# neuronika/neuronika

Hardware: AMD Instinct MI355X
Metric: training-step samples/sec (fwd+bwd+allreduce) (higher is better)
Workload: dtype f32

## Files before the change

neuronika_amd/csrc/nk_gemm.hip:

```cpp
#include "nk_mma.h"
#include <utility>

using namespace nkmma;

static bool aligned16(const void* p) { return (reinterpret_cast<uintptr_t>(p) & 15) == 0; }
constexpr int GEMM_CHAIN_K = 2048;
constexpr int PF2_MIN_KTILES = 48;

struct GemmArgs {
    const float* A;
    const float* B;
    float* C;
    int M, N, K;
    long long lda, ldb, ldc;
    float alpha, beta;
    const float* bias;
    int relu;
    const float* mask;
    long long ldm;
    int batch_inner;
    long long sAo, sAi, sBo, sBi, sCo, sCi;
    int splits;
    int k_per_split;
    float* slabs;
    int tiles_m, tiles_n;
    int chunk;
    int group_m;
    int pf2_min;
    int kskew;
};

template <bool ALIGNED, int TI, int TJ, bool EPX>
__device__ __forceinline__ void gemm_epilogue(const GemmArgs& p, f32x16 (&acc)[TI][TJ], int m0, int n0, int bo, int bi, int split,
                                              int batch, int wr, int wc, int lane) {
    if (p.splits > 1) {
        float* S = p.slabs + ((long long)split * gridDim.z + batch) * (long long)p.M * p.N;
        const int M = p.M, N = p.N;
        acc_foreach<TI, TJ>(acc, wr, wc, lane, [&](int r, int c, float v) {
            const int row = m0 + r, col = n0 + c;
            if (ALIGNED || (row < M && col < N)) S[(long long)row * N + col] = v;
        });
        return;
    }
    float* C = p.C + bo * p.sCo + bi * p.sCi;
    const float alpha = p.alpha, beta = p.beta;
    const int M = p.M, N = p.N;
    const long long ldc = p.ldc;
    if (EPX && p.mask != nullptr) {
        const float* Mk = p.mask;
        const long long ldm = p.ldm;
#pragma unroll
        for (int i = 0; i < TI; ++i)
#pragma unroll
            for (int j = 0; j < TJ; ++j) {
                float mv[16], old[16];
#pragma unroll
                for (int e = 0; e < 16; ++e) {
                    const int row = m0 + (wr * TI + i) * 32 + (e & 3) + 8 * (e >> 2) + 4 * (lane >> 5), col = n0 + (wc * TJ + j) * 32 + (lane & 31);
                    const bool ok = ALIGNED || (row < M && col < N);
                    mv[e] = ok ? Mk[row * ldm + col] : 0.f;
                    old[e] = (ok && beta != 0.f) ? C[row * ldc + col] : 0.f;
                }
#pragma unroll
                for (int e = 0; e < 16; ++e) {
                    const int row = m0 + (wr * TI + i) * 32 + (e & 3) + 8 * (e >> 2) + 4 * (lane >> 5), col = n0 + (wc * TJ + j) * 32 + (lane & 31);
                    float o = alpha * acc[i][j][e];
                    o = mv[e] > 0.f ? o : 0.f * o;
                    if (ALIGNED || (row < M && col < N)) C[row * ldc + col] = beta == 0.f ? o : fmaf(beta, old[e], o);
                }
            }
        return;
    }
    if (p.bias != nullptr || beta != 0.f || alpha != 1.f || (EPX && p.relu)) {
        float old[TI][TJ][16];
        if (beta != 0.f)
            acc_foreach_idx<TI, TJ>(acc, wr, wc, lane, [&](int i, int j, int e, int r, int c, float) {
                const int row = m0 + r, col = n0 + c;
                old[i][j][e] = (ALIGNED || (row < M && col < N)) ? C[row * ldc + col] : 0.f;
            });
        float bv[TJ];
#pragma unroll
        for (int j = 0; j < TJ; ++j) {
            const int col = n0 + (wc * TJ + j) * 32 + (lane & 31);
            bv[j] = (p.bias != nullptr && (ALIGNED || col < N)) ? p.bias[col] : 0.f;
        }
        const bool relu = EPX && p.relu != 0;
#pragma unroll
        for (int i = 0; i < TI; ++i)
#pragma unroll
            for (int j = 0; j < TJ; ++j)
#pragma unroll
                for (int e = 0; e < 16; ++e) {
                    float o = alpha * acc[i][j][e];
                    if (p.bias != nullptr) o += bv[j];
                    if constexpr (EPX) o = relu ? fmaxf(o, 0.f) : o;
                    acc[i][j][e] = beta == 0.f ? o : fmaf(beta, old[i][j][e], o);
                }
    }
    acc_foreach<TI, TJ>(acc, wr, wc, lane, [&](int r, int c, float v) {
        const int row = m0 + r, col = n0 + c;
        if (ALIGNED || (row < M && col < N)) C[row * ldc + col] = v;
    });
}

template <bool AKC, bool BKC, bool ALIGNED, int TI, int TJ, int KG>
__device__ __forceinline__ void gemm_loop_lookahead2(TileLoader<AKC, 64 * TI>& la, TileLoader<BKC, 64 * TJ>& lb, f32x16 (&acc)[TI][TJ],
                                                     float* smem, int nt, bool skew, int t, int wr, int wc, int lane) {
    constexpr int BM = 64 * TI, BN = 64 * TJ;
    constexpr int TA_FLOATS = tile_floats<AKC, BM>(), STAGE = TA_FLOATS + tile_floats<BKC, BN>();
    float* const buf0 = smem;
    float* const buf1 = smem + STAGE;
    Stage<BM / 32> pa, qa;
    Stage<BN / 32> pb, qb;
    if (nt > 0) {
        pa = la.template load<ALIGNED>(t);
        pb = lb.template load<ALIGNED>(t);
        stage_store<AKC, BM>(buf0, pa, t);
        stage_store<BKC, BN>(buf0 + TA_FLOATS, pb, t);
    }
    __syncthreads();
    if (nt > 1) {
        pa = la.template load<ALIGNED>(t);
        pb = lb.template load<ALIGNED>(t);
    }
    int it = 0;
    for (; it + 3 < nt; it += 2) {
        if (KG == 2 && skew) {
            mma_tile<AKC, BKC, TI, TJ, 0, BK / 16>(buf0, buf0 + TA_FLOATS, acc, wr, wc, lane);
            __builtin_amdgcn_sched_barrier(0);
        }
        qa = la.template load<ALIGNED>(t);
        qb = lb.template load<ALIGNED>(t);
        stage_store<AKC, BM>(buf1, pa, t);
        stage_store<BKC, BN>(buf1 + TA_FLOATS, pb, t);
        __builtin_amdgcn_sched_barrier(0);
        if (KG == 2 && skew) mma_tile<AKC, BKC, TI, TJ, BK / 16, BK / 8>(buf0, buf0 + TA_FLOATS, acc, wr, wc, lane);
        else mma_tile<AKC, BKC, TI, TJ>(buf0, buf0 + TA_FLOATS, acc, wr, wc, lane);
        __syncthreads();
        if (KG == 2 && skew) {
            mma_tile<AKC, BKC, TI, TJ, 0, BK / 16>(buf1, buf1 + TA_FLOATS, acc, wr, wc, lane);
            __builtin_amdgcn_sched_barrier(0);
        }
        pa = la.template load<ALIGNED>(t);
        pb = lb.template load<ALIGNED>(t);
        stage_store<AKC, BM>(buf0, qa, t);
        stage_store<BKC, BN>(buf0 + TA_FLOATS, qb, t);
        __builtin_amdgcn_sched_barrier(0);
        if (KG == 2 && skew) mma_tile<AKC, BKC, TI, TJ, BK / 16, BK / 8>(buf1, buf1 + TA_FLOATS, acc, wr, wc, lane);
        else mma_tile<AKC, BKC, TI, TJ>(buf1, buf1 + TA_FLOATS, acc, wr, wc, lane);
        __syncthreads();
    }
    const int left = nt - it;
    if (left == 3) {
        qa = la.template load<ALIGNED>(t);
        qb = lb.template load<ALIGNED>(t);
    }
    if (left >= 2) {
        stage_store<AKC, BM>(buf1, pa, t);
        stage_store<BKC, BN>(buf1 + TA_FLOATS, pb, t);
    }
    if (left >= 1) mma_tile<AKC, BKC, TI, TJ>(buf0, buf0 + TA_FLOATS, acc, wr, wc, lane);
    if (left >= 2) {
        __syncthreads();
        if (left == 3) {
            stage_store<AKC, BM>(buf0, qa, t);
            stage_store<BKC, BN>(buf0 + TA_FLOATS, qb, t);
        }
        mma_tile<AKC, BKC, TI, TJ>(buf1, buf1 + TA_FLOATS, acc, wr, wc, lane);
        if (left == 3) {
            __syncthreads();
            mma_tile<AKC, BKC, TI, TJ>(buf0, buf0 + TA_FLOATS, acc, wr, wc, lane);
        }
    }
}

template <bool TA, bool TB, int TI, int TJ, int KG>
constexpr int gemm_smem_floats() { return KG * 2 * (tile_floats<!TA, 64 * TI>() + tile_floats<TB, 64 * TJ>()); }

template <bool TA, bool TB, bool ALIGNED, int TI, int TJ, int KG = 1, bool EPX = false>
__global__ __launch_bounds__(NT * KG, (min_waves<TI, TJ, !TA && TB>())) void sgemm_kernel(GemmArgs p) {
    __shared__ __attribute__((aligned(16))) float smem_all[gemm_smem_floats<TA, TB, TI, TJ, KG>()];
#define NK_GEMM_BX blockIdx.x
#define NK_GEMM_NBX gridDim.x
#define NK_GEMM_SPLIT blockIdx.y
#include "nk_gemm_body.h"
#undef NK_GEMM_BX
#undef NK_GEMM_NBX
#undef NK_GEMM_SPLIT
}

template <bool TA, bool TB, bool ALIGNED, int TI, int TJ, int KG, bool EPX>
__device__ __forceinline__ void sgemm_body(const GemmArgs& p, float* smem_all, int bx, int nbx) {
#define NK_GEMM_BX bx
#define NK_GEMM_NBX nbx
#define NK_GEMM_SPLIT blockIdx.y
#include "nk_gemm_body.h"
#undef NK_GEMM_BX
#undef NK_GEMM_NBX
#undef NK_GEMM_SPLIT
}
template <bool TA, bool TB, bool ALIGNED, int TI, int TJ, int KG, bool EPX>
__device__ __forceinline__ void sgemm_body_split(const GemmArgs& p, float* smem_all, int bx, int nbx, int split_no) {
#define NK_GEMM_BX bx
#define NK_GEMM_NBX nbx
#define NK_GEMM_SPLIT split_no
#include "nk_gemm_body.h"
#undef NK_GEMM_BX
#undef NK_GEMM_NBX
#undef NK_GEMM_SPLIT
}

struct GemmPairArgs {
    GemmArgs p0, p1;
    int nblk0;
};
template <bool TA0, bool TB0, bool TA1, bool TB1, int TI, int TJ>
__global__ __launch_bounds__(NT, (min_waves<TI, TJ, (!TA0 && TB0) || (!TA1 && TB1)>())) void sgemm_pair_kernel(GemmPairArgs pp) {
    constexpr int F0 = gemm_smem_floats<TA0, TB0, TI, TJ, 1>(), F1 = gemm_smem_floats<TA1, TB1, TI, TJ, 1>();
    __shared__ __attribute__((aligned(16))) float smem_all[F0 > F1 ? F0 : F1];
    const int nblk0 = pp.nblk0;
    if ((int)blockIdx.x < nblk0)
        sgemm_body<TA0, TB0, true, TI, TJ, 1, false>(pp.p0, smem_all, blockIdx.x, nblk0);
    else
        sgemm_body<TA1, TB1, true, TI, TJ, 1, false>(pp.p1, smem_all, blockIdx.x - nblk0, gridDim.x - nblk0);
}

struct GemmTailArgs {
    GemmArgs p0, p1;
    int nfull, ntail;
};
template <bool TA, bool TB, bool EPX>
__global__ __launch_bounds__(NT, (min_waves<2, 2, !TA && TB>())) void sgemm_tail_kernel(GemmTailArgs pp) {
    __shared__ __attribute__((aligned(16))) float smem_all[gemm_smem_floats<TA, TB, 2, 2, 1>()];
    const int nfull = pp.nfull;
    if ((int)blockIdx.x < nfull) {
        sgemm_body_split<TA, TB, true, 2, 2, 1, EPX>(pp.p0, smem_all, blockIdx.x, nfull, 0);
    } else {
        const int r = (int)blockIdx.x - nfull, ntail = pp.ntail;
        sgemm_body_split<TA, TB, true, 2, 2, 1, false>(pp.p1, smem_all, r % ntail, ntail, r / ntail);
    }
}

__global__ void splitk_reduce_kernel(const float* __restrict__ slabs, float* __restrict__ C, int M, int N,
                                     long long ldc, int splits, int nbatch, int batch_inner,
                                     long long sCo, long long sCi, float alpha, float beta,
                                     const float* __restrict__ bias, int relu, const float* __restrict__ mask, long long ldm) {
    const long long per = (long long)M * N;
    const long long total = per * nbatch;
    for (long long i = blockIdx.x * (long long)blockDim.x + threadIdx.x; i < total;
         i += (long long)gridDim.x * blockDim.x) {
        const int b = (int)(i / per);
        const long long e = i % per;
        const int row = (int)(e / N), col = (int)(e % N);
        float s = 0.f;
        for (int k = 0; k < splits; ++k) s += slabs[((long long)k * nbatch + b) * per + e];
        float* q = C + (b / batch_inner) * sCo + (b % batch_inner) * sCi + row * ldc + col;
        float o = alpha * s;
        if (mask) o = mask[row * ldm + col] > 0.f ? o : 0.f * o;
        if (bias) o += bias[col];
        if (relu) o = fmaxf(o, 0.f);
        *q = beta == 0.f ? o : fmaf(beta, *q, o);
    }
}

__global__ void splitk_reduce_flat_kernel(const float* __restrict__ slabs, float* __restrict__ C, long long total4, int splits,
                                          float alpha, float beta, const float* __restrict__ bias, int N, int relu,
                                          const float* __restrict__ mask) {
    for (long long i = blockIdx.x * (long long)blockDim.x + threadIdx.x; i < total4; i += (long long)gridDim.x * blockDim.x) {
        float4 s = make_float4(0.f, 0.f, 0.f, 0.f);
        for (int k = 0; k < splits; ++k) {
            const float4 v = reinterpret_cast<const float4*>(slabs)[(long long)k * total4 + i];
            s.x += v.x; s.y += v.y; s.z += v.z; s.w += v.w;
        }
        float4 o = make_float4(alpha * s.x, alpha * s.y, alpha * s.z, alpha * s.w);
        if (mask) {
            const float4 m = reinterpret_cast<const float4*>(mask)[i];
            o.x = m.x > 0.f ? o.x : 0.f * o.x; o.y = m.y > 0.f ? o.y : 0.f * o.y; o.z = m.z > 0.f ? o.z : 0.f * o.z; o.w = m.w > 0.f ? o.w : 0.f * o.w;
        }
        if (bias) {
            const int col = (int)((i * 4) % N);
            const float4 b = *reinterpret_cast<const float4*>(bias + col);
            o.x += b.x; o.y += b.y; o.z += b.z; o.w += b.w;
        }
        if (relu) { o.x = fmaxf(o.x, 0.f); o.y = fmaxf(o.y, 0.f); o.z = fmaxf(o.z, 0.f); o.w = fmaxf(o.w, 0.f); }
        float4* q = reinterpret_cast<float4*>(C) + i;
        if (beta != 0.f) { const float4 c = *q; o.x = fmaf(beta, c.x, o.x); o.y = fmaf(beta, c.y, o.y); o.z = fmaf(beta, c.z, o.z); o.w = fmaf(beta, c.w, o.w); }
        *q = o;
    }
}


template <bool TA, bool TB, int TI, int TJ, bool EPX>
static int launch_tile(nk_device* dev, const GemmArgs& p, int nbatch, bool aligned, int kg = 1) {
    dim3 grid((p.tiles_m * p.tiles_n + p.chunk - 1) / p.chunk, p.splits, nbatch), block(NT * kg);
    if constexpr (TI * TJ == 4 || TI * TJ == 1) {
        if (kg == 2) {
            hipLaunchKernelGGL((sgemm_kernel<TA, TB, true, TI, TJ, 2, EPX>), grid, block, 0, dev->compute, p);
            NK_LAUNCH_CHECK();
            return NK_OK;
        }
    }
    if (aligned)
        hipLaunchKernelGGL((sgemm_kernel<TA, TB, true, TI, TJ, 1, EPX>), grid, block, 0, dev->compute, p);
    else
        hipLaunchKernelGGL((sgemm_kernel<TA, TB, false, TI, TJ, 1, EPX>), grid, block, 0, dev->compute, p);
    NK_LAUNCH_CHECK();
    return NK_OK;
}

template <bool TA, bool TB, bool EPX>
static int launch_epx(nk_device* dev, const GemmArgs& p, int nbatch, bool aligned, int ti, int tj, int kg) {
    if (ti == 2 && tj == 2) return launch_tile<TA, TB, 2, 2, EPX>(dev, p, nbatch, aligned, kg);
    if (ti == 2 && tj == 1) return launch_tile<TA, TB, 2, 1, EPX>(dev, p, nbatch, aligned);
    if (ti == 1 && tj == 2) return launch_tile<TA, TB, 1, 2, EPX>(dev, p, nbatch, aligned);
    return launch_tile<TA, TB, 1, 1, EPX>(dev, p, nbatch, aligned, kg);
}
template <bool TA, bool TB>
static int launch(nk_device* dev, const GemmArgs& p, int nbatch, bool aligned, int ti, int tj, int kg) {
    if constexpr (!TA && TB) {
        return launch_epx<TA, TB, true>(dev, p, nbatch, aligned, ti, tj, kg);
    } else if constexpr (TA) {
        NK_CHECK(!p.relu && p.mask == nullptr, "GEMM with a transposed A has no ReLU / mask epilogue");
        return launch_epx<TA, TB, false>(dev, p, nbatch, aligned, ti, tj, kg);
    } else {
        const bool epx = p.relu || p.mask != nullptr;
        return epx ? launch_epx<TA, TB, true>(dev, p, nbatch, aligned, ti, tj, kg) : launch_epx<TA, TB, false>(dev, p, nbatch, aligned, ti, tj, kg);
    }
}

struct GemmPlan {
    GemmArgs p;
    int ti, tj, kg, nbatch;
    bool aligned, empty;
};

static int gemm_plan(nk_device* dev, int transA, int transB, int M, int N, int K, float alpha,
                     const float* A, int lda, long long sAo, long long sAi, const float* B, int ldb,
                     long long sBo, long long sBi, float beta, float* C, int ldc, long long sCo,
                     long long sCi, int batch_outer, int batch_inner, const float* bias, int relu,
                     const float* mask, long long ldm, GemmPlan* plan, bool allow_kpair = true) {
    NK_USE(dev);
    NK_CHECK(M >= 0 && N >= 0 && K >= 0 && batch_outer >= 0 && batch_inner >= 0, "negative GEMM extent");
    const int nbatch = batch_outer * batch_inner;
    plan->empty = M == 0 || N == 0 || nbatch == 0;
    plan->nbatch = nbatch;
    if (plan->empty) return NK_OK;
    NK_CHECK(A && B && C, "null GEMM operand");
    NK_CHECK(lda >= (transA ? M : K) && ldb >= (transB ? K : N) && ldc >= N,
             "leading dimension too small (lda=%d ldb=%d ldc=%d)", lda, ldb, ldc);
    NK_CHECK(nbatch <= 65535, "batch count %d exceeds grid.z", nbatch);

    GemmArgs p{};
    p.A = A; p.B = B; p.C = C;
    p.M = M; p.N = N; p.K = K;
    p.lda = lda; p.ldb = ldb; p.ldc = ldc;
    p.alpha = alpha; p.beta = beta;
    p.bias = bias;
    p.relu = relu; p.mask = mask; p.ldm = ldm;
    NK_CHECK(mask == nullptr || (nbatch == 1 && ldm >= N), "masked GEMM: one matrix, ldm >= N");
    NK_CHECK(!transA || (!relu && mask == nullptr), "GEMM with a transposed A has no ReLU / mask epilogue");
    p.batch_inner = batch_inner;
    p.sAo = sAo; p.sAi = sAi; p.sBo = sBo; p.sBi = sBi; p.sCo = sCo; p.sCi = sCi;

    auto blocks = [&](int ti, int tj) {
        return (long long)((M + 64 * ti - 1) / (64 * ti)) * ((N + 64 * tj - 1) / (64 * tj)) * nbatch;
    };
    const int ktiles = (K + BK - 1) / BK;
    int ti = (M <= 64 || (M % 128 != 0 && M % 64 == 0)) ? 1 : 2;
    int tj = (N <= 64 || (N % 128 != 0 && N % 64 == 0)) ? 1 : 2;
    int splits = 1;
    if (blocks(ti, tj) >= 512) {
        auto wave_eff = [&](long long nb, long long slots) { return (double)nb / (double)(((nb + slots - 1) / slots) * slots); };
        const int ti0 = ti, tj0 = tj;
        double best = (ti0 * tj0 == 4 ? 1.0 : ti0 * tj0 == 2 ? 0.9 : 0.8) * wave_eff(blocks(ti0, tj0), ti0 * tj0 == 4 ? 512 : 768);
        if (ti0 * tj0 == 4) {
            const double c21 = 0.9 * wave_eff(blocks(2, 1), 768), c12 = 0.9 * wave_eff(blocks(1, 2), 768);
            if (c12 > best + 0.05) { best = c12; ti = 1; tj = 2; }
            if (c21 > best + 0.05) { best = c21; ti = 2; tj = 1; }
        }
        if (ti0 * tj0 >= 2) {
            const long long nb1 = blocks(1, 1);
            double q = wave_eff(nb1, 768);
            if (nb1 >= 1536 && q < 0.9) q = 0.9;
            if (0.8 * q > best + 0.05) { ti = 1; tj = 1; }
        }
    } else if (blocks(ti, tj) < 512) {
        const long long nb = blocks(ti, tj);
        long long s = (512 + nb - 1) / nb;
        if (s > ktiles / 16) s = ktiles / 16;
        if (ti * tj == 4 && nb >= 256 && ktiles >= PF2_MIN_KTILES) {
            splits = 1;
        } else if (ti * tj > 1 && s >= 1 && nb * s >= 384) {
            splits = (int)s;
        } else {
            ti = tj = 1;
            const long long nb1 = blocks(1, 1);
            if (nb1 < 256) {
                s = 512 / nb1;
                if (s > ktiles / 8) s = ktiles / 8;
                splits = s < 1 ? 1 : (int)s;
            }
        }
    }
    p.tiles_m = (M + 64 * ti - 1) / (64 * ti);
    p.tiles_n = (N + 64 * tj - 1) / (64 * tj);
    int force_chunk = 0, force_group = 0, force_pf2 = 0;
    if (dev->tune_gemm_n >= 3 && (dev->tune_gemm[0] == 1 || dev->tune_gemm[0] == 2) && (dev->tune_gemm[1] == 1 || dev->tune_gemm[1] == 2)) {
        ti = dev->tune_gemm[0]; tj = dev->tune_gemm[1]; splits = dev->tune_gemm[2] < 1 ? 1 : dev->tune_gemm[2];
        p.tiles_m = (M + 64 * ti - 1) / (64 * ti);
        p.tiles_n = (N + 64 * tj - 1) / (64 * tj);
        if (dev->tune_gemm_n >= 4) force_chunk = dev->tune_gemm[3];
        if (dev->tune_gemm_n >= 5) force_group = dev->tune_gemm[4];
        if (dev->tune_gemm_n >= 6) force_pf2 = dev->tune_gemm[5];
    }
    if (splits > 1 && dev->tune_gemm_n < 3 && splits < (ktiles + 127) / 128) splits = (ktiles + 127) / 128;
    int kts = (ktiles + splits - 1) / splits;
    if (kts < 1) kts = 1;
    splits = (ktiles + kts - 1) / kts;
    if (splits < 1) splits = 1;
    p.splits = splits;
    p.k_per_split = kts * BK;
    const int pf2_rule_for_chunk = ti * tj == 1 ? 8 : ((!transA && !transB) ? 32 : PF2_MIN_KTILES);
    {
        const long long ntiles = (long long)p.tiles_m * p.tiles_n, slots = ti * tj == 4 ? 512 : (ti * tj == 2 ? 768 : 1024);
        long long c = kts >= 16 ? 1 : (16 + kts - 1) / kts;
        const long long cap = ntiles * splits * nbatch / (4 * slots);
        if (c > cap) c = cap;
        if (c > ntiles) c = ntiles;
        const int pf2_effective = force_pf2 > 0 ? force_pf2 : pf2_rule_for_chunk;
        if (c < 1 || kts >= 8) c = 1;
        if (force_chunk > 0) c = force_chunk;
        if (kts >= pf2_effective) c = 1;
        p.chunk = (int)c;
    }
    p.group_m = force_group > 0 ? force_group : 8;
    const int pf2_rule = ti * tj == 1 ? 8 : ((!transA && !transB) ? 32 : PF2_MIN_KTILES);
    p.pf2_min = force_pf2 > 0 ? force_pf2 : pf2_rule;

    const int BM = 64 * ti, BN = 64 * tj;
    const bool aligned = (M % BM == 0) && (N % BN == 0) && (K % BK == 0) && (lda % 4 == 0) &&
                         (ldb % 4 == 0) && aligned16(A) && aligned16(B) && (sAo % 4 == 0) &&
                         (sAi % 4 == 0) && (sBo % 4 == 0) && (sBi % 4 == 0);
    const int kpair_tune = allow_kpair ? dev->tune_kpair : 0;
    int kg = 1;
    p.kskew = 1;
    {
        const long long nblk = (long long)p.tiles_m * p.tiles_n * p.splits * nbatch;
        const bool can = (ti * tj == 4 || ti * tj == 1) && aligned && p.chunk == 1 && kts % 2 == 0 && kts >= 8 && K % (2 * BK) == 0 &&
                         (p.splits == 1 || p.k_per_split * p.splits == K);
        const bool want = kpair_tune >= 0 ? kpair_tune > 0 : nblk <= dev->num_cus && kts >= (ti * tj == 4 ? 32 : 16);
        if (can && want) kg = 2;
        if (kpair_tune == 1) p.kskew = 0;
    }
    plan->p = p; plan->ti = ti; plan->tj = tj; plan->kg = kg; plan->aligned = aligned;
    return NK_OK;
}

template <bool TA, bool TB>
static void launch_tail(nk_device* dev, const GemmTailArgs& pp, dim3 grid, bool epx) {
    if constexpr (!TA && TB) {
        hipLaunchKernelGGL((sgemm_tail_kernel<TA, TB, true>), grid, dim3(NT), 0, dev->compute, pp);
    } else if constexpr (TA) {
        hipLaunchKernelGGL((sgemm_tail_kernel<TA, TB, false>), grid, dim3(NT), 0, dev->compute, pp);
    } else {
        if (epx) hipLaunchKernelGGL((sgemm_tail_kernel<TA, TB, true>), grid, dim3(NT), 0, dev->compute, pp);
        else hipLaunchKernelGGL((sgemm_tail_kernel<TA, TB, false>), grid, dim3(NT), 0, dev->compute, pp);
    }
}
static int gemm_tail_launch(nk_device* dev, int transA, int transB, const GemmArgs& p, bool* taken) {
    *taken = false;
    const long long T = (long long)p.tiles_m * p.tiles_n;
    const long long slots = 2LL * dev->num_cus - dev->busy_slots;
    if (slots < dev->num_cus || T <= slots || T % slots == 0) return NK_OK;
    const int gsize = p.tiles_m % p.group_m == 0 ? p.group_m : p.tiles_m % p.group_m;
    long long tail = T % slots;
    tail = (tail + gsize - 1) / gsize * gsize;
    if (tail > (long long)gsize * p.tiles_n || tail >= T) return NK_OK;
    const int ktiles = p.K / BK;
    long long pieces = slots / tail;
    if (pieces < 4) return NK_OK;
    int kts = (int)((ktiles + pieces - 1) / pieces);
    if (kts < 4) kts = 4;
    const int s_eff = (ktiles + kts - 1) / kts;
    if (s_eff < 2) return NK_OK;
    const int cols = (int)(tail / gsize);
    const int m_lo = (p.tiles_m - gsize) * 128, n_lo = (p.tiles_n - cols) * 128;
    const int Ms = p.M - m_lo, Ns = p.N - n_lo;
    void* ws = nullptr;
    int rc = nk_workspace(dev, (size_t)s_eff * Ms * Ns * sizeof(float), &ws);
    if (rc) return rc;
    GemmTailArgs pp;
    pp.p0 = p;
    pp.p1 = p;
    GemmArgs& q = pp.p1;
    q.A = p.A + (transA ? (long long)m_lo : (long long)m_lo * p.lda);
    q.B = p.B + (transB ? (long long)n_lo * p.ldb : (long long)n_lo);
    q.C = p.C + (long long)m_lo * p.ldc + n_lo;
    q.M = Ms; q.N = Ns;
    q.tiles_m = gsize; q.tiles_n = cols;
    q.splits = s_eff; q.k_per_split = kts * BK; q.slabs = (float*)ws;
    q.bias = nullptr; q.relu = 0; q.mask = nullptr;
    pp.nfull = (int)(T - tail);
    pp.ntail = (int)tail;
    rc = nk_prof_start(dev, NK_KERNEL_SGEMM, 2.0 * p.M * p.N * (double)p.K);
    if (rc) return rc;
    const dim3 grid((unsigned)(pp.nfull + tail * s_eff), 1, 1);
    const bool epx = p.relu || p.mask != nullptr || (!transA && transB);
    if (!transA && !transB) launch_tail<false, false>(dev, pp, grid, epx);
    else if (!transA && transB) launch_tail<false, true>(dev, pp, grid, epx);
    else launch_tail<true, false>(dev, pp, grid, epx);
    NK_LAUNCH_CHECK();
    hipLaunchKernelGGL(splitk_reduce_kernel, dim3(nk_stream_grid((size_t)Ms * Ns, 256)), dim3(256), 0, dev->compute, q.slabs, q.C, Ms, Ns,
                       p.ldc, s_eff, 1, 1, 0LL, 0LL, p.alpha, p.beta, p.bias ? p.bias + n_lo : nullptr, p.relu,
                       p.mask ? p.mask + (long long)m_lo * p.ldm + n_lo : nullptr, p.ldm);
    NK_LAUNCH_CHECK();
    *taken = true;
    return nk_prof_stop(dev);
}

static int gemm_impl(nk_device* dev, int transA, int transB, int M, int N, int K, float alpha,
                     const float* A, int lda, long long sAo, long long sAi, const float* B, int ldb,
                     long long sBo, long long sBi, float beta, float* C, int ldc, long long sCo,
                     long long sCi, int batch_outer, int batch_inner, const float* bias = nullptr, int relu = 0,
                     const float* mask = nullptr, long long ldm = 0, bool allow_kpair = true, bool allow_chain = true) {
    GemmPlan plan;
    int rc = gemm_plan(dev, transA, transB, M, N, K, alpha, A, lda, sAo, sAi, B, ldb, sBo, sBi, beta, C, ldc, sCo, sCi, batch_outer,
                       batch_inner, bias, relu, mask, ldm, &plan, allow_kpair);
    if (rc || plan.empty) return rc;
    {
        const long long chain = dev->tune_chain < 0 ? GEMM_CHAIN_K : dev->tune_chain;
        const long long reach = chain * plan.kg;
        if (allow_chain && chain > 0 && K > reach && plan.p.splits == 1 && !bias && !relu && !mask && dev->tune_gemm_n < 3) {
            const int pieces = (int)((K + reach - 1) / reach);
            const int per = ((K + pieces - 1) / pieces + 2 * BK - 1) / (2 * BK) * (2 * BK);
            for (int k0 = 0; k0 < K && !rc; k0 += per) {
                const int kk = K - k0 < per ? K - k0 : per;
                rc = gemm_impl(dev, transA, transB, M, N, kk, alpha, A + (transA ? (long long)k0 * lda : (long long)k0), lda, sAo, sAi,
                               B + (transB ? (long long)k0 : (long long)k0 * ldb), ldb, sBo, sBi, k0 == 0 ? beta : 1.f, C, ldc, sCo, sCi,
                               batch_outer, batch_inner, nullptr, 0, nullptr, 0, allow_kpair, false);
            }
            return rc;
        }
    }
    GemmArgs& p = plan.p;
    const int nbatch = plan.nbatch, ti = plan.ti, tj = plan.tj, kg = plan.kg;
    const bool aligned = plan.aligned;
    if (dev->busy_slots > 0 && ti == 2 && tj == 2 && kg == 1 && aligned && p.splits == 1 && p.chunk == 1 && nbatch == 1 &&
        !(transA && transB) && dev->tune_gemm_n < 3) {
        bool taken = false;
        rc = gemm_tail_launch(dev, transA, transB, p, &taken);
        if (rc || taken) return rc;
    }
    if (p.splits > 1) {
        void* ws = nullptr;
        rc = nk_workspace(dev, (size_t)p.splits * nbatch * M * N * sizeof(float), &ws);
        if (rc) return rc;
        p.slabs = (float*)ws;
    }
    rc = nk_prof_start(dev, NK_KERNEL_SGEMM, 2.0 * M * N * (double)K * nbatch);
    if (rc) return rc;
    if (!transA && !transB) rc = launch<false, false>(dev, p, nbatch, aligned, ti, tj, kg);
    else if (!transA && transB) rc = launch<false, true>(dev, p, nbatch, aligned, ti, tj, kg);
    else if (transA && !transB) rc = launch<true, false>(dev, p, nbatch, aligned, ti, tj, kg);
    else rc = launch<true, true>(dev, p, nbatch, aligned, ti, tj, kg);
    if (rc) return rc;
    if (p.splits > 1) {
        const long long total = (long long)M * N * nbatch;
        const bool dense = ldc == N && N % 4 == 0 && aligned16(C) && (!bias || aligned16(bias)) && (!mask || (ldm == N && aligned16(mask))) &&
                           (nbatch == 1 || (sCi == (long long)M * N && (batch_outer == 1 || sCo == (long long)batch_inner * M * N)));
        if (dense)
            hipLaunchKernelGGL(splitk_reduce_flat_kernel, dim3(nk_stream_grid((size_t)(total / 4), 256)), dim3(256), 0, dev->compute,
                               p.slabs, C, total / 4, p.splits, alpha, beta, bias, N, relu, mask);
        else
        hipLaunchKernelGGL(splitk_reduce_kernel, dim3(nk_stream_grid((size_t)total, 256)), dim3(256), 0,
                           dev->compute, p.slabs, C, M, N, (long long)ldc, p.splits, nbatch, batch_inner,
                           sCo, sCi, alpha, beta, bias, relu, mask, ldm);
        NK_LAUNCH_CHECK();
    }
    return nk_prof_stop(dev);
}

struct GemmProblem {
    int transA, transB, M, N, K;
    const float* A; int lda; long long sAo, sAi;
    const float* B; int ldb; long long sBo, sBi;
    float beta; float* C; int ldc; long long sCo, sCi;
};

template <bool TA0, bool TB0>
static int launch_pair(nk_device* dev, const GemmPairArgs& pp, dim3 grid, int ti, int tj) {
    if (ti == 2 && tj == 2) hipLaunchKernelGGL((sgemm_pair_kernel<TA0, TB0, true, false, 2, 2>), grid, dim3(NT), 0, dev->compute, pp);
    else if (ti == 2 && tj == 1) hipLaunchKernelGGL((sgemm_pair_kernel<TA0, TB0, true, false, 2, 1>), grid, dim3(NT), 0, dev->compute, pp);
    else hipLaunchKernelGGL((sgemm_pair_kernel<TA0, TB0, true, false, 1, 1>), grid, dim3(NT), 0, dev->compute, pp);
    NK_LAUNCH_CHECK();
    return NK_OK;
}

static int gemm_pair_impl(nk_device* dev, const GemmProblem& a, const GemmProblem& b, int batch_outer, int batch_inner) {
    NK_USE(dev);
    auto alone = [&](const GemmProblem& q) {
        return gemm_impl(dev, q.transA, q.transB, q.M, q.N, q.K, 1.f, q.A, q.lda, q.sAo, q.sAi, q.B, q.ldb, q.sBo, q.sBi, q.beta, q.C, q.ldc,
                         q.sCo, q.sCi, batch_outer, batch_inner, nullptr, 0, nullptr, 0, false);
    };
    auto two_launches = [&]() { const int rc = alone(a); return rc ? rc : alone(b); };
    const int mode = dev->tune_pair;
    if (mode == 0) return two_launches();
    GemmPlan q0, q1;
    int rc = gemm_plan(dev, a.transA, a.transB, a.M, a.N, a.K, 1.f, a.A, a.lda, a.sAo, a.sAi, a.B, a.ldb, a.sBo, a.sBi, a.beta, a.C, a.ldc,
                       a.sCo, a.sCi, batch_outer, batch_inner, nullptr, 0, nullptr, 0, &q0, false);
    if (!rc)
        rc = gemm_plan(dev, b.transA, b.transB, b.M, b.N, b.K, 1.f, b.A, b.lda, b.sAo, b.sAi, b.B, b.ldb, b.sBo, b.sBi, b.beta, b.C, b.ldc,
                       b.sCo, b.sCi, batch_outer, batch_inner, nullptr, 0, nullptr, 0, &q1, false);
    if (rc) return rc;
    if (q0.empty || q1.empty) return two_launches();
    {
        const long long chain = dev->tune_chain < 0 ? GEMM_CHAIN_K : dev->tune_chain;
        if (chain > 0 && dev->tune_gemm_n < 3 && ((a.K > chain && q0.p.splits == 1) || (b.K > chain && q1.p.splits == 1))) return two_launches();
    }
    const long long batch = (long long)batch_outer * batch_inner;
    {
        struct Foot { const float* p; long long rows, width, ld; bool ok; };
        auto foot = [&](const float* p, long long rows, long long cols, long long ld, long long so, long long si) {
            Foot f{p, rows, cols, ld, true};
            if (batch_inner > 1) {
                if (si < ld) f.width = cols + (batch_inner - 1) * si;
                else if (si % ld == 0) f.rows = rows + (batch_inner - 1) * (si / ld);
                else f.ok = false;
            }
            if (batch_outer > 1) {
                if (so % ld == 0) f.rows += (batch_outer - 1) * (so / ld);
                else f.ok = false;
            }
            if (f.width > ld) f.ok = false;
            if (!f.ok) { f.rows = 1; f.ld = 0; f.width = (batch_outer - 1) * so + (batch_inner - 1) * si + (rows - 1) * ld + cols; }
            return f;
        };
        auto opnd = [&](const GemmProblem& q, int which) {
            if (which == 0) return foot(q.A, q.transA ? q.K : q.M, q.transA ? q.M : q.K, q.lda, q.sAo, q.sAi);
            if (which == 1) return foot(q.B, q.transB ? q.N : q.K, q.transB ? q.K : q.N, q.ldb, q.sBo, q.sBi);
            return foot(q.C, q.M, q.N, q.ldc, q.sCo, q.sCi);
        };
        auto hits = [](const Foot& x, const Foot& y) {
            const uintptr_t x0 = (uintptr_t)x.p, x1 = (uintptr_t)(x.p + (x.rows - 1) * x.ld + x.width);
            const uintptr_t y0 = (uintptr_t)y.p, y1 = (uintptr_t)(y.p + (y.rows - 1) * y.ld + y.width);
            if (!(x0 < y1 && y0 < x1)) return false;
            if (x.ok && y.ok && x.ld == y.ld && x.ld > 0) {
                const long long ld = x.ld, r = ((y.p - x.p) % ld + ld) % ld;
                if (r >= x.width && r + y.width <= ld) return false;
            }
            return true;
        };
        bool clash = false;
        for (int w = 0; w < 3; ++w) clash = clash || hits(opnd(a, 2), opnd(b, w)) || hits(opnd(b, 2), opnd(a, w));
        if (clash) return two_launches();
    }
    const bool layouts = !(a.transA && a.transB) && b.transA && !b.transB;
    const bool tiles = q0.ti == q1.ti && q0.tj == q1.tj && (q0.ti == q0.tj || (q0.ti == 2 && q0.tj == 1));
    const bool plain = q0.aligned && q1.aligned && q0.p.splits == 1 && q1.p.splits == 1 && q0.p.chunk == 1 && q1.p.chunk == 1;
    if (!(layouts && tiles && plain)) return two_launches();
    const long long nblk0 = (long long)q0.p.tiles_m * q0.p.tiles_n, nblk1 = (long long)q1.p.tiles_m * q1.p.tiles_n;
    if (nblk0 + nblk1 > 0x7fffffffLL) return two_launches();
    if (mode < 0) {
        const int per_cu = q0.ti * q0.tj == 4 ? 2 : (q0.ti * q0.tj == 2 ? ((!a.transA && a.transB) ? 2 : 3) : 4);
        if ((nblk0 + nblk1) * batch > (long long)dev->num_cus * per_cu) return two_launches();
    }
    GemmPairArgs pp;
    pp.p0 = q0.p; pp.p1 = q1.p; pp.nblk0 = (int)nblk0;
    rc = nk_prof_start(dev, NK_KERNEL_SGEMM, 2.0 * batch * ((double)a.M * a.N * a.K + (double)b.M * b.N * b.K));
    if (rc) return rc;
    const dim3 grid((unsigned)(nblk0 + nblk1), 1, (unsigned)batch);
    if (a.transA) rc = launch_pair<true, false>(dev, pp, grid, q0.ti, q0.tj);
    else if (a.transB) rc = launch_pair<false, true>(dev, pp, grid, q0.ti, q0.tj);
    else rc = launch_pair<false, false>(dev, pp, grid, q0.ti, q0.tj);
    if (rc) return rc;
    return nk_prof_stop(dev);
}

extern "C" {

int nk_sgemm(nk_device* dev, int transA, int transB, int M, int N, int K, float alpha, const float* A,
             int lda, const float* B, int ldb, float beta, float* C, int ldc) {
    return gemm_impl(dev, transA, transB, M, N, K, alpha, A, lda, 0, 0, B, ldb, 0, 0, beta, C, ldc, 0, 0, 1, 1);
}

int nk_sgemm_batched(nk_device* dev, int transA, int transB, int M, int N, int K, float alpha,
                     const float* A, int lda, long long sAo, long long sAi, const float* B, int ldb,
                     long long sBo, long long sBi, float beta, float* C, int ldc, long long sCo,
                     long long sCi, int batch_outer, int batch_inner) {
    return gemm_impl(dev, transA, transB, M, N, K, alpha, A, lda, sAo, sAi, B, ldb, sBo, sBi, beta, C, ldc,
                     sCo, sCi, batch_outer, batch_inner);
}

int nk_mm_fwd(nk_device* dev, const float* A, const float* B, float* C, int n, int m, int o) {
    return nk_sgemm(dev, 0, 0, n, o, m, 1.f, A, m, B, o, 0.f, C, o);
}
static int node_bwd_product(nk_device* dev, int transA, int transB, int M, int N, int K, const float* A, int lda, const float* B, int ldb,
                            float* C, int ldc) {
    return gemm_impl(dev, transA, transB, M, N, K, 1.f, A, lda, 0, 0, B, ldb, 0, 0, 1.f, C, ldc, 0, 0, 1, 1, nullptr, 0, nullptr, 0, false);
}
int nk_mm_bwd_left(nk_device* dev, float* dA, const float* G, const float* B, int n, int m, int o) {
    return node_bwd_product(dev, 0, 1, n, m, o, G, o, B, o, dA, m);
}
int nk_mm_bwd_right(nk_device* dev, float* dB, const float* A, const float* G, int n, int m, int o) {
    return node_bwd_product(dev, 1, 0, m, o, n, A, m, G, o, dB, o);
}
int nk_sgemm_pair(nk_device* dev, int transA0, int transB0, int M0, int N0, int K0, const float* A0, int lda0, const float* B0, int ldb0,
                  float beta0, float* C0, int ldc0, int transA1, int transB1, int M1, int N1, int K1, const float* A1, int lda1,
                  const float* B1, int ldb1, float beta1, float* C1, int ldc1) {
    const GemmProblem a{transA0, transB0, M0, N0, K0, A0, lda0, 0, 0, B0, ldb0, 0, 0, beta0, C0, ldc0, 0, 0};
    const GemmProblem b{transA1, transB1, M1, N1, K1, A1, lda1, 0, 0, B1, ldb1, 0, 0, beta1, C1, ldc1, 0, 0};
    return gemm_pair_impl(dev, a, b, 1, 1);
}
int nk_sgemm_pair_batched(nk_device* dev, int batch_outer, int batch_inner,
                          int transA0, int transB0, int M0, int N0, int K0, const float* A0, int lda0, long long sA0o, long long sA0i,
                          const float* B0, int ldb0, long long sB0o, long long sB0i, float beta0, float* C0, int ldc0, long long sC0o, long long sC0i,
                          int transA1, int transB1, int M1, int N1, int K1, const float* A1, int lda1, long long sA1o, long long sA1i,
                          const float* B1, int ldb1, long long sB1o, long long sB1i, float beta1, float* C1, int ldc1, long long sC1o, long long sC1i) {
    const GemmProblem a{transA0, transB0, M0, N0, K0, A0, lda0, sA0o, sA0i, B0, ldb0, sB0o, sB0i, beta0, C0, ldc0, sC0o, sC0i};
    const GemmProblem b{transA1, transB1, M1, N1, K1, A1, lda1, sA1o, sA1i, B1, ldb1, sB1o, sB1i, beta1, C1, ldc1, sC1o, sC1i};
    return gemm_pair_impl(dev, a, b, batch_outer, batch_inner);
}
int nk_mm_bwd(nk_device* dev, float* dA, float* dB, const float* G, const float* A, const float* B, int n, int m, int o, int assign_a,
              int assign_b) {
    return nk_sgemm_pair(dev, 0, 1, n, m, o, G, o, B, o, assign_a ? 0.f : 1.f, dA, m, 1, 0, m, o, n, A, m, G, o, assign_b ? 0.f : 1.f, dB, o);
}
int nk_mm_t_bwd(nk_device* dev, float* dA, float* dB, const float* G, const float* A, const float* B, int n, int m, int o, int assign_a,
                int assign_b) {
    return nk_sgemm_pair(dev, 0, 0, n, m, o, G, o, B, m, assign_a ? 0.f : 1.f, dA, m, 1, 0, o, m, n, G, o, A, m, assign_b ? 0.f : 1.f, dB, m);
}
int nk_mm_t_fwd(nk_device* dev, const float* A, const float* B, float* C, int n, int m, int o) {
    return nk_sgemm(dev, 0, 1, n, o, m, 1.f, A, m, B, m, 0.f, C, o);
}
int nk_linear_fwd(nk_device* dev, const float* X, const float* W, const float* bias, float* Y, int n, int m, int o) {
    NK_CHECK(bias != nullptr, "null bias");
    return gemm_impl(dev, 0, 1, n, o, m, 1.f, X, m, 0, 0, W, m, 0, 0, 0.f, Y, o, 0, 0, 1, 1, bias);
}
int nk_linear_relu_fwd(nk_device* dev, const float* X, const float* W, const float* bias, float* Y, int n, int m, int o) {
    NK_CHECK(bias != nullptr, "null bias");
    return gemm_impl(dev, 0, 1, n, o, m, 1.f, X, m, 0, 0, W, m, 0, 0, 0.f, Y, o, 0, 0, 1, 1, bias, 1);
}
int nk_linear_bwd_input_relu(nk_device* dev, float* dX, const float* G, const float* W, const float* X, int n, int m, int o, int assign) {
    NK_CHECK(X != nullptr, "null mask operand");
    return gemm_impl(dev, 0, 0, n, m, o, 1.f, G, o, 0, 0, W, m, 0, 0, assign ? 0.f : 1.f, dX, m, 0, 0, 1, 1, nullptr, 0, X, m);
}
int nk_mm_t_bwd_left(nk_device* dev, float* dA, const float* G, const float* B, int n, int m, int o) {
    return node_bwd_product(dev, 0, 0, n, m, o, G, o, B, m, dA, m);
}
int nk_mm_t_bwd_right(nk_device* dev, float* dB, const float* G, const float* A, int n, int m, int o) {
    return node_bwd_product(dev, 1, 0, o, m, n, G, o, A, m, dB, m);
}

}
```

neuronika_amd/csrc/nk_mma.h:

```cpp
#pragma once
#include "nk_common.h"

namespace nkmma {

using f32x16 = __attribute__((ext_vector_type(16))) float;
typedef float f32x4u __attribute__((ext_vector_type(4), aligned(4)));

constexpr int BK = 32;
constexpr int NT = 256;
constexpr int LDK = BK + 4;

template <bool KC, int R>
constexpr int tile_floats() { return KC ? R * LDK : R * BK; }
template <int TI, int TJ, bool BOTH_KC = false>
constexpr int min_waves() { return TI * TJ == 4 ? 2 : (TI * TJ == 2 ? (BOTH_KC ? 2 : 3) : 4); }

template <int NV>
struct Stage;
template <>
struct Stage<4> {
    float4 v0, v1, v2, v3;
};
template <>
struct Stage<2> {
    float4 v0, v1;
};

__device__ __forceinline__ int kc_row(int idx) { return ((idx >> 7) << 4) + (((idx >> 3) & 1) << 3) + ((idx >> 4) & 7); }
__device__ __forceinline__ int kc_q(int idx) { return idx & 7; }

template <bool KC, int R>
__device__ __forceinline__ int lds_slot(int idx) {
    return KC ? kc_row(idx) * LDK + kc_q(idx) * 4 : (idx / (R / 4)) * R + (idx % (R / 4)) * 4;
}

template <bool KC, int R>
__device__ __forceinline__ void stage_store(float* Xs, const Stage<R / 32>& r, int t) {
    *reinterpret_cast<float4*>(&Xs[lds_slot<KC, R>(t)]) = r.v0;
    *reinterpret_cast<float4*>(&Xs[lds_slot<KC, R>(t + NT)]) = r.v1;
    if constexpr (R == 128) {
        *reinterpret_cast<float4*>(&Xs[lds_slot<KC, R>(t + 2 * NT)]) = r.v2;
        *reinterpret_cast<float4*>(&Xs[lds_slot<KC, R>(t + 3 * NT)]) = r.v3;
    }
}

template <bool KC, int R>
struct TileLoader {
    const float* base;
    long long kstep;
    unsigned o0, o1, o2, o3;
    const float* X;
    long long ld;
    int row0, rows, kend, k0;
    bool interior;

    __device__ __forceinline__ void init(const float* X_, long long ld_, int row0_, int k0_, int rows_,
                                         int kend_, int t) {
        X = X_; ld = ld_; row0 = row0_; rows = rows_; kend = kend_; k0 = k0_;
        interior = row0_ + R <= rows_;
        base = KC ? X_ + (long long)row0_ * ld_ + k0_ : X_ + (long long)k0_ * ld_ + row0_;
        kstep = KC ? BK : (long long)BK * ld_;
        o0 = off(t, ld_); o1 = off(t + NT, ld_); o2 = off(t + 2 * NT, ld_); o3 = off(t + 3 * NT, ld_);
    }
    static __device__ __forceinline__ unsigned off(int idx, long long ld_) {
        return KC ? (unsigned)(kc_row(idx) * ld_ + kc_q(idx) * 4)
                  : (unsigned)((idx / (R / 4)) * ld_ + (idx % (R / 4)) * 4);
    }
    __device__ __forceinline__ float4 guarded(int idx) const {
        float v[4];
        if (KC) {
            const int row = row0 + kc_row(idx), k = k0 + kc_q(idx) * 4;
#pragma unroll
            for (int c = 0; c < 4; ++c) v[c] = (row < rows && k + c < kend) ? X[row * ld + k + c] : 0.f;
        } else {
            const int k = k0 + idx / (R / 4), row = row0 + (idx % (R / 4)) * 4;
#pragma unroll
            for (int c = 0; c < 4; ++c) v[c] = (k < kend && row + c < rows) ? X[k * ld + row + c] : 0.f;
        }
        return make_float4(v[0], v[1], v[2], v[3]);
    }
    template <bool ALIGNED>
    __device__ __forceinline__ Stage<R / 32> load(int t) {
        Stage<R / 32> r;
        if (ALIGNED) {
            r.v0 = *reinterpret_cast<const float4*>(base + o0);
            r.v1 = *reinterpret_cast<const float4*>(base + o1);
            if constexpr (R == 128) {
                r.v2 = *reinterpret_cast<const float4*>(base + o2);
                r.v3 = *reinterpret_cast<const float4*>(base + o3);
            }
            base += kstep;
        } else if (interior && k0 + BK <= kend) {
#define NK_LDU(V, O) { const f32x4u q = *reinterpret_cast<const f32x4u*>(base + O); V = make_float4(q.x, q.y, q.z, q.w); }
            NK_LDU(r.v0, o0) NK_LDU(r.v1, o1)
            if constexpr (R == 128) { NK_LDU(r.v2, o2) NK_LDU(r.v3, o3) }
#undef NK_LDU
            base += kstep;
            k0 += BK;
        } else {
            r.v0 = guarded(t);
            r.v1 = guarded(t + NT);
            if constexpr (R == 128) {
                r.v2 = guarded(t + 2 * NT);
                r.v3 = guarded(t + 3 * NT);
            }
            base += kstep;
            k0 += BK;
        }
        return r;
    }
};

template <bool KC, int R>
__device__ __forceinline__ void frag_read(float (&f)[4], const float* Xs, int rowbase, int k8, int lane) {
    const int r = lane & 31, h = lane >> 5;
    if (KC) {
        const float4 v = *reinterpret_cast<const float4*>(&Xs[(rowbase + r) * LDK + k8 + 4 * h]);
        f[0] = v.x; f[1] = v.y; f[2] = v.z; f[3] = v.w;
    } else {
#pragma unroll
        for (int i = 0; i < 4; ++i) f[i] = Xs[(k8 + 4 * h + i) * R + rowbase + r];
    }
}

template <bool AKC, bool BKC, int TI, int TJ, int G0 = 0, int G1 = BK / 8>
__device__ __forceinline__ void mma_tile(const float* As, const float* Bs, f32x16 (&acc)[TI][TJ], int wr, int wc,
                                         int lane) {
    float a[2][TI][4], b[2][TJ][4];
#pragma unroll
    for (int i = 0; i < TI; ++i) frag_read<AKC, 64 * TI>(a[G0 & 1][i], As, (wr * TI + i) * 32, G0 * 8, lane);
#pragma unroll
    for (int j = 0; j < TJ; ++j) frag_read<BKC, 64 * TJ>(b[G0 & 1][j], Bs, (wc * TJ + j) * 32, G0 * 8, lane);
#pragma unroll
    for (int g = G0; g < G1; ++g) {
        const int cb = g & 1, nb = cb ^ 1;
        if (g + 1 < G1) {
#pragma unroll
            for (int i = 0; i < TI; ++i) frag_read<AKC, 64 * TI>(a[nb][i], As, (wr * TI + i) * 32, (g + 1) * 8, lane);
#pragma unroll
            for (int j = 0; j < TJ; ++j) frag_read<BKC, 64 * TJ>(b[nb][j], Bs, (wc * TJ + j) * 32, (g + 1) * 8, lane);
            __builtin_amdgcn_sched_barrier(0);
        }
#pragma unroll
        for (int s = 0; s < 4; ++s)
#pragma unroll
            for (int i = 0; i < TI; ++i)
#pragma unroll
                for (int j = 0; j < TJ; ++j)
                    acc[i][j] = __builtin_amdgcn_mfma_f32_32x32x2f32(a[cb][i][s], b[cb][j][s], acc[i][j], 0, 0, 0);
    }
}

template <int TI, int TJ>
__device__ __forceinline__ void acc_zero(f32x16 (&acc)[TI][TJ]) {
#pragma unroll
    for (int i = 0; i < TI; ++i)
#pragma unroll
        for (int j = 0; j < TJ; ++j)
#pragma unroll
            for (int e = 0; e < 16; ++e) acc[i][j][e] = 0.f;
}

template <int TI, int TJ, class F>
__device__ __forceinline__ void acc_foreach(const f32x16 (&acc)[TI][TJ], int wr, int wc, int lane, F&& f) {
    const int c = lane & 31, h = lane >> 5;
#pragma unroll
    for (int i = 0; i < TI; ++i)
#pragma unroll
        for (int j = 0; j < TJ; ++j)
#pragma unroll
            for (int e = 0; e < 16; ++e) {
                const int row = (wr * TI + i) * 32 + (e & 3) + 8 * (e >> 2) + 4 * h;
                const int col = (wc * TJ + j) * 32 + c;
                f(row, col, acc[i][j][e]);
            }
}

template <int TI, int TJ, class FC, class FE>
__device__ __forceinline__ void acc_foreach_cols(const f32x16 (&acc)[TI][TJ], int wr, int wc, int lane, FC&& fc, FE&& fe) {
    const int c = lane & 31, h = lane >> 5;
#pragma unroll
    for (int j = 0; j < TJ; ++j) {
        const auto ctx = fc((wc * TJ + j) * 32 + c);
#pragma unroll
        for (int i = 0; i < TI; ++i)
#pragma unroll
            for (int e = 0; e < 16; ++e) fe((wr * TI + i) * 32 + (e & 3) + 8 * (e >> 2) + 4 * h, ctx, acc[i][j][e]);
    }
}

__device__ __forceinline__ void pin_regs(float4& q) { asm volatile("" : "+v"(q.x), "+v"(q.y), "+v"(q.z), "+v"(q.w)); }

template <int TI, int TJ, class F>
__device__ __forceinline__ void acc_foreach_idx(const f32x16 (&acc)[TI][TJ], int wr, int wc, int lane, F&& f) {
    const int c = lane & 31, h = lane >> 5;
#pragma unroll
    for (int i = 0; i < TI; ++i)
#pragma unroll
        for (int j = 0; j < TJ; ++j)
#pragma unroll
            for (int e = 0; e < 16; ++e)
                f(i, j, e, (wr * TI + i) * 32 + (e & 3) + 8 * (e >> 2) + 4 * h, (wc * TJ + j) * 32 + c, acc[i][j][e]);
}
template <int TI, int TJ, class FC, class FE>
__device__ __forceinline__ void acc_foreach_cols_idx(const f32x16 (&acc)[TI][TJ], int wr, int wc, int lane, FC&& fc, FE&& fe) {
    const int c = lane & 31, h = lane >> 5;
#pragma unroll
    for (int j = 0; j < TJ; ++j) {
        const auto ctx = fc((wc * TJ + j) * 32 + c);
#pragma unroll
        for (int i = 0; i < TI; ++i)
#pragma unroll
            for (int e = 0; e < 16; ++e) fe(i, j, e, (wr * TI + i) * 32 + (e & 3) + 8 * (e >> 2) + 4 * h, ctx, acc[i][j][e]);
    }
}

__device__ __forceinline__ int xcd_chunk(int bid, int nblk) {
    constexpr int NXCD = 8;
    const int q = nblk / NXCD, rem = nblk % NXCD;
    const int xcd = bid % NXCD, loc = bid / NXCD;
    return (xcd < rem ? xcd * (q + 1) : rem * (q + 1) + (xcd - rem) * q) + loc;
}
__device__ __forceinline__ void tile_of_seq(int swz, int tiles_m, int tiles_n, int& tm, int& tn, int GROUP_M = 8) {
    const int per_group = GROUP_M * tiles_n;
    const int group = swz / per_group;
    const int first_m = group * GROUP_M;
    const int gsize = min(tiles_m - first_m, GROUP_M);
    const int in_group = swz % per_group;
    tm = first_m + in_group % gsize;
    tn = in_group / gsize;
}
__device__ __forceinline__ void tile_coords(int bid, int nblk, int tiles_m, int tiles_n, int& tm, int& tn) {
    constexpr int NXCD = 8;
    const int q = nblk / NXCD, rem = nblk % NXCD;
    const int xcd = bid % NXCD, loc = bid / NXCD;
    const int swz = (xcd < rem ? xcd * (q + 1) : rem * (q + 1) + (xcd - rem) * q) + loc;
    constexpr int GROUP_M = 8;
    const int per_group = GROUP_M * tiles_n;
    const int group = swz / per_group;
    const int first_m = group * GROUP_M;
    const int gsize = min(tiles_m - first_m, GROUP_M);
    const int in_group = swz % per_group;
    tm = first_m + in_group % gsize;
    tn = in_group / gsize;
}

}
```

Before: 489,400.

## Carry first k-group fragments across stage barrier in single-group GEMM mainloop

For the non-split-K (KG==1) GEMM path, the mainloop now moves the block barrier inside the MFMA tile loop, just before the last k-group's MFMAs. Right after it, the first fragment group of the next shared-memory stage is read into carried registers. This overlaps the LDS fragment read latency at each stage boundary with the remaining MFMAs instead of stalling at the start of each tile. It costs extra registers for the carried fragments, which can lower occupancy, and the tail handling becomes more intricate.

```diff
diff --git a/neuronika_amd/csrc/nk_gemm.hip b/neuronika_amd/csrc/nk_gemm.hip
--- a/neuronika_amd/csrc/nk_gemm.hip
+++ b/neuronika_amd/csrc/nk_gemm.hip
@@ -123,54 +123,93 @@
         pa = la.template load<ALIGNED>(t);
         pb = lb.template load<ALIGNED>(t);
     }
+    if constexpr (KG == 2) {
+        int it = 0;
+        for (; it + 3 < nt; it += 2) {
+            if (KG == 2 && skew) {
+                mma_tile<AKC, BKC, TI, TJ, 0, BK / 16>(buf0, buf0 + TA_FLOATS, acc, wr, wc, lane);
+                __builtin_amdgcn_sched_barrier(0);
+            }
+            qa = la.template load<ALIGNED>(t);
+            qb = lb.template load<ALIGNED>(t);
+            stage_store<AKC, BM>(buf1, pa, t);
+            stage_store<BKC, BN>(buf1 + TA_FLOATS, pb, t);
+            __builtin_amdgcn_sched_barrier(0);
+            if (KG == 2 && skew) mma_tile<AKC, BKC, TI, TJ, BK / 16, BK / 8>(buf0, buf0 + TA_FLOATS, acc, wr, wc, lane);
+            else mma_tile<AKC, BKC, TI, TJ>(buf0, buf0 + TA_FLOATS, acc, wr, wc, lane);
+            __syncthreads();
+            if (KG == 2 && skew) {
+                mma_tile<AKC, BKC, TI, TJ, 0, BK / 16>(buf1, buf1 + TA_FLOATS, acc, wr, wc, lane);
+                __builtin_amdgcn_sched_barrier(0);
+            }
+            pa = la.template load<ALIGNED>(t);
+            pb = lb.template load<ALIGNED>(t);
+            stage_store<AKC, BM>(buf0, qa, t);
+            stage_store<BKC, BN>(buf0 + TA_FLOATS, qb, t);
+            __builtin_amdgcn_sched_barrier(0);
+            if (KG == 2 && skew) mma_tile<AKC, BKC, TI, TJ, BK / 16, BK / 8>(buf1, buf1 + TA_FLOATS, acc, wr, wc, lane);
+            else mma_tile<AKC, BKC, TI, TJ>(buf1, buf1 + TA_FLOATS, acc, wr, wc, lane);
+            __syncthreads();
+        }
+        const int left = nt - it;
+        if (left == 3) {
+            qa = la.template load<ALIGNED>(t);
+            qb = lb.template load<ALIGNED>(t);
+        }
+        if (left >= 2) {
+            stage_store<AKC, BM>(buf1, pa, t);
+            stage_store<BKC, BN>(buf1 + TA_FLOATS, pb, t);
+        }
+        if (left >= 1) mma_tile<AKC, BKC, TI, TJ>(buf0, buf0 + TA_FLOATS, acc, wr, wc, lane);
+        if (left >= 2) {
+            __syncthreads();
+            if (left == 3) {
+                stage_store<AKC, BM>(buf0, qa, t);
+                stage_store<BKC, BN>(buf0 + TA_FLOATS, qb, t);
+            }
+            mma_tile<AKC, BKC, TI, TJ>(buf1, buf1 + TA_FLOATS, acc, wr, wc, lane);
+            if (left == 3) {
+                __syncthreads();
+                mma_tile<AKC, BKC, TI, TJ>(buf0, buf0 + TA_FLOATS, acc, wr, wc, lane);
+            }
+        }
+    } else {
+    float ca[TI][4], cb[TJ][4];
+    if (nt > 0) frag_read_group<AKC, BKC, TI, TJ>(ca, cb, buf0, buf0 + TA_FLOATS, 0, wr, wc, lane);
     int it = 0;
     for (; it + 3 < nt; it += 2) {
-        if (KG == 2 && skew) {
-            mma_tile<AKC, BKC, TI, TJ, 0, BK / 16>(buf0, buf0 + TA_FLOATS, acc, wr, wc, lane);
-            __builtin_amdgcn_sched_barrier(0);
-        }
         qa = la.template load<ALIGNED>(t);
         qb = lb.template load<ALIGNED>(t);
         stage_store<AKC, BM>(buf1, pa, t);
         stage_store<BKC, BN>(buf1 + TA_FLOATS, pb, t);
         __builtin_amdgcn_sched_barrier(0);
-        if (KG == 2 && skew) mma_tile<AKC, BKC, TI, TJ, BK / 16, BK / 8>(buf0, buf0 + TA_FLOATS, acc, wr, wc, lane);
-        else mma_tile<AKC, BKC, TI, TJ>(buf0, buf0 + TA_FLOATS, acc, wr, wc, lane);
-        __syncthreads();
-        if (KG == 2 && skew) {
-            mma_tile<AKC, BKC, TI, TJ, 0, BK / 16>(buf1, buf1 + TA_FLOATS, acc, wr, wc, lane);
-            __builtin_amdgcn_sched_barrier(0);
-        }
+        mma_tile_carry<AKC, BKC, TI, TJ, true>(buf0, buf0 + TA_FLOATS, buf1, buf1 + TA_FLOATS, acc, ca, cb, wr, wc, lane);
         pa = la.template load<ALIGNED>(t);
         pb = lb.template load<ALIGNED>(t);
         stage_store<AKC, BM>(buf0, qa, t);
         stage_store<BKC, BN>(buf0 + TA_FLOATS, qb, t);
         __builtin_amdgcn_sched_barrier(0);
-        if (KG == 2 && skew) mma_tile<AKC, BKC, TI, TJ, BK / 16, BK / 8>(buf1, buf1 + TA_FLOATS, acc, wr, wc, lane);
-        else mma_tile<AKC, BKC, TI, TJ>(buf1, buf1 + TA_FLOATS, acc, wr, wc, lane);
-        __syncthreads();
+        mma_tile_carry<AKC, BKC, TI, TJ, true>(buf1, buf1 + TA_FLOATS, buf0, buf0 + TA_FLOATS, acc, ca, cb, wr, wc, lane);
     }
     const int left = nt - it;
     if (left == 3) {
         qa = la.template load<ALIGNED>(t);
         qb = lb.template load<ALIGNED>(t);
     }
+    const float* last = buf0;
     if (left >= 2) {
         stage_store<AKC, BM>(buf1, pa, t);
         stage_store<BKC, BN>(buf1 + TA_FLOATS, pb, t);
-    }
-    if (left >= 1) mma_tile<AKC, BKC, TI, TJ>(buf0, buf0 + TA_FLOATS, acc, wr, wc, lane);
-    if (left >= 2) {
-        __syncthreads();
+        mma_tile_carry<AKC, BKC, TI, TJ, true>(buf0, buf0 + TA_FLOATS, buf1, buf1 + TA_FLOATS, acc, ca, cb, wr, wc, lane);
         if (left == 3) {
             stage_store<AKC, BM>(buf0, qa, t);
             stage_store<BKC, BN>(buf0 + TA_FLOATS, qb, t);
-        }
-        mma_tile<AKC, BKC, TI, TJ>(buf1, buf1 + TA_FLOATS, acc, wr, wc, lane);
-        if (left == 3) {
-            __syncthreads();
-            mma_tile<AKC, BKC, TI, TJ>(buf0, buf0 + TA_FLOATS, acc, wr, wc, lane);
-        }
+            mma_tile_carry<AKC, BKC, TI, TJ, true>(buf1, buf1 + TA_FLOATS, buf0, buf0 + TA_FLOATS, acc, ca, cb, wr, wc, lane);
+        } else {
+            last = buf1;
+        }
+    }
+    if (left >= 1) mma_tile_carry<AKC, BKC, TI, TJ, false>(last, last + TA_FLOATS, last, last + TA_FLOATS, acc, ca, cb, wr, wc, lane);
     }
 }
 
diff --git a/neuronika_amd/csrc/nk_mma.h b/neuronika_amd/csrc/nk_mma.h
--- a/neuronika_amd/csrc/nk_mma.h
+++ b/neuronika_amd/csrc/nk_mma.h
@@ -151,6 +151,53 @@
     }
 }
 
+template <bool AKC, bool BKC, int TI, int TJ>
+__device__ __forceinline__ void frag_read_group(float (&a)[TI][4], float (&b)[TJ][4], const float* As, const float* Bs, int g,
+                                                int wr, int wc, int lane) {
+#pragma unroll
+    for (int i = 0; i < TI; ++i) frag_read<AKC, 64 * TI>(a[i], As, (wr * TI + i) * 32, g * 8, lane);
+#pragma unroll
+    for (int j = 0; j < TJ; ++j) frag_read<BKC, 64 * TJ>(b[j], Bs, (wc * TJ + j) * 32, g * 8, lane);
+}
+
+template <bool AKC, bool BKC, int TI, int TJ, bool NEXT, int POS = 3 * (BK / 8)>
+__device__ __forceinline__ void mma_tile_carry(const float* As, const float* Bs, const float* An, const float* Bn,
+                                               f32x16 (&acc)[TI][TJ], float (&ca)[TI][4], float (&cb)[TJ][4], int wr, int wc,
+                                               int lane) {
+    constexpr int NG = BK / 8;
+    static_assert(POS > 4 * (NG - 2) && POS < 4 * NG, "the barrier lies behind the read of the last k-group");
+    float a[2][TI][4], b[2][TJ][4];
+#pragma unroll
+    for (int s = 0; s < 4; ++s) {
+#pragma unroll
+        for (int i = 0; i < TI; ++i) a[0][i][s] = ca[i][s];
+#pragma unroll
+        for (int j = 0; j < TJ; ++j) b[0][j][s] = cb[j][s];
+    }
+#pragma unroll
+    for (int g = 0; g < NG; ++g) {
+        const int cur = g & 1, nb = cur ^ 1;
+        if (g + 1 < NG) {
+            frag_read_group<AKC, BKC, TI, TJ>(a[nb], b[nb], As, Bs, g + 1, wr, wc, lane);
+            __builtin_amdgcn_sched_barrier(0);
+        }
+#pragma unroll
+        for (int s = 0; s < 4; ++s) {
+            if (NEXT && g * 4 + s == POS) {
+                __builtin_amdgcn_sched_barrier(0);
+                __syncthreads();
+                frag_read_group<AKC, BKC, TI, TJ>(ca, cb, An, Bn, 0, wr, wc, lane);
+                __builtin_amdgcn_sched_barrier(0);
+            }
+#pragma unroll
+            for (int i = 0; i < TI; ++i)
+#pragma unroll
+                for (int j = 0; j < TJ; ++j)
+                    acc[i][j] = __builtin_amdgcn_mfma_f32_32x32x2f32(a[cur][i][s], b[cur][j][s], acc[i][j], 0, 0, 0);
+        }
+    }
+}
+
 template <int TI, int TJ>
 __device__ __forceinline__ void acc_zero(f32x16 (&acc)[TI][TJ]) {
 #pragma unroll
```

New measurement: 482,100. -1.5%, worse.
